# WanqingXia/UR-gym

Hardware: AMD Instinct MI355X
Metric: env-steps/sec (whole node) (higher is better)
Workload: dtype f64; 1 GPU; UR5DynReach-v1 N=65536 per GPU, random actions U(-1,1), auto-reset, seed 0; envs_total=65536, gather_obs=False, rollout_api=False, gjk_start=bullet

## Files before the change

ur_gym_amd/csrc/urgym_device.h:

```cpp
#pragma once
#include <stdint.h>
#if defined(URGYM_HOST_HARNESS)
#include <cmath>
#define __device__
#define __forceinline__ inline
#define URGYM_LDS
static inline uint32_t __umulhi(uint32_t a, uint32_t b) { return (uint32_t)(((uint64_t)a * b) >> 32); }
using std::fma; using std::sqrt; using std::fabs; using std::fmin; using std::fmax; using std::acos; using std::asin; using std::atan2;
#else
#include <hip/hip_runtime.h>
#define URGYM_LDS __attribute__((address_space(3)))
#endif
#include "urgym_philox.h"

namespace urgym {

struct D3 {
  double x, y, z;
};
__device__ __forceinline__ D3 d3(double x, double y, double z) { return D3{x, y, z}; }
__device__ __forceinline__ D3 operator+(D3 a, D3 b) { return d3(a.x + b.x, a.y + b.y, a.z + b.z); }
__device__ __forceinline__ D3 operator-(D3 a, D3 b) { return d3(a.x - b.x, a.y - b.y, a.z - b.z); }
__device__ __forceinline__ D3 operator-(D3 a) { return d3(-a.x, -a.y, -a.z); }
__device__ __forceinline__ D3 operator*(D3 a, double s) { return d3(a.x * s, a.y * s, a.z * s); }
__device__ __forceinline__ double dot(D3 a, D3 b) { return fma(a.x, b.x, fma(a.y, b.y, a.z * b.z)); }
__device__ __forceinline__ D3 cross(D3 a, D3 b) {
  return d3(a.y * b.z - a.z * b.y, a.z * b.x - a.x * b.z, a.x * b.y - a.y * b.x);
}
__device__ __forceinline__ double len2(D3 a) { return dot(a, a); }
__device__ __forceinline__ D3 sel(bool c, D3 a, D3 b) { return d3(c ? a.x : b.x, c ? a.y : b.y, c ? a.z : b.z); }

struct X3 {
  double r[9];
  D3 t;
};
__device__ __forceinline__ D3 rot(const X3& T, D3 v) {
  return d3(fma(T.r[0], v.x, fma(T.r[1], v.y, T.r[2] * v.z)), fma(T.r[3], v.x, fma(T.r[4], v.y, T.r[5] * v.z)),
            fma(T.r[6], v.x, fma(T.r[7], v.y, T.r[8] * v.z)));
}
__device__ __forceinline__ D3 rotT(const X3& T, D3 v) {
  return d3(fma(T.r[0], v.x, fma(T.r[3], v.y, T.r[6] * v.z)), fma(T.r[1], v.x, fma(T.r[4], v.y, T.r[7] * v.z)),
            fma(T.r[2], v.x, fma(T.r[5], v.y, T.r[8] * v.z)));
}
__device__ __forceinline__ D3 apply(const X3& T, D3 v) { return rot(T, v) + T.t; }
__device__ __forceinline__ X3 rel(const X3& A, const X3& B) {
  X3 C;
#pragma unroll
  for (int i = 0; i < 3; i++)
#pragma unroll
    for (int j = 0; j < 3; j++) C.r[i * 3 + j] = fma(A.r[i], B.r[j], fma(A.r[3 + i], B.r[3 + j], A.r[6 + i] * B.r[6 + j]));
  C.t = rotT(A, B.t - A.t);
  return C;
}

struct XRef {
  URGYM_LDS double* p;
  int stride;
  __device__ __forceinline__ double at(int k) const { return p[k * stride]; }
  __device__ __forceinline__ void set(int k, double v) const { p[k * stride] = v; }
};
__device__ __forceinline__ void store(XRef R, const X3& T) {
#pragma unroll
  for (int k = 0; k < 9; k++) R.set(k, T.r[k]);
  R.set(9, T.t.x); R.set(10, T.t.y); R.set(11, T.t.z);
}
__device__ __forceinline__ D3 rotT(XRef T, D3 v) {
  return d3(fma(T.at(0), v.x, fma(T.at(3), v.y, T.at(6) * v.z)), fma(T.at(1), v.x, fma(T.at(4), v.y, T.at(7) * v.z)),
            fma(T.at(2), v.x, fma(T.at(5), v.y, T.at(8) * v.z)));
}
__device__ __forceinline__ D3 apply(XRef T, D3 v) {
  return d3(fma(T.at(0), v.x, fma(T.at(1), v.y, T.at(2) * v.z)) + T.at(9), fma(T.at(3), v.x, fma(T.at(4), v.y, T.at(5) * v.z)) + T.at(10),
            fma(T.at(6), v.x, fma(T.at(7), v.y, T.at(8) * v.z)) + T.at(11));
}

struct Q4 {
  double x, y, z, w;
};
__device__ __forceinline__ Q4 qmul(Q4 a, Q4 b) {
  return Q4{a.w * b.x + a.x * b.w + a.y * b.z - a.z * b.y, a.w * b.y + a.y * b.w + a.z * b.x - a.x * b.z,
            a.w * b.z + a.z * b.w + a.x * b.y - a.y * b.x, a.w * b.w - a.x * b.x - a.y * b.y - a.z * b.z};
}
__device__ __forceinline__ void quat_to_rot(Q4 q, double r[9]) {
  double d = q.x * q.x + q.y * q.y + q.z * q.z + q.w * q.w;
  double s = 2.0 / d;
  double xs = q.x * s, ys = q.y * s, zs = q.z * s;
  double wx = q.w * xs, wy = q.w * ys, wz = q.w * zs, xx = q.x * xs, xy = q.x * ys, xz = q.x * zs;
  double yy = q.y * ys, yz = q.y * zs, zz = q.z * zs;
  r[0] = 1.0 - (yy + zz); r[1] = xy - wz; r[2] = xz + wy;
  r[3] = xy + wz; r[4] = 1.0 - (xx + zz); r[5] = yz - wx;
  r[6] = xz - wy; r[7] = yz + wx; r[8] = 1.0 - (xx + yy);
}
__device__ __forceinline__ Q4 rot_to_quat(const double r[9]) {
  double tr = r[0] + r[4] + r[8];
  Q4 q;
  if (tr > 0.0) {
    double s = sqrt(tr + 1.0);
    q.w = 0.5 * s;
    s = 0.5 / s;
    q.x = (r[7] - r[5]) * s; q.y = (r[2] - r[6]) * s; q.z = (r[3] - r[1]) * s;
  } else if (r[0] >= r[4] && r[0] >= r[8]) {
    double s = sqrt(r[0] - r[4] - r[8] + 1.0);
    q.x = 0.5 * s;
    s = 0.5 / s;
    q.w = (r[7] - r[5]) * s; q.y = (r[3] + r[1]) * s; q.z = (r[6] + r[2]) * s;
  } else if (r[4] >= r[8]) {
    double s = sqrt(r[4] - r[8] - r[0] + 1.0);
    q.y = 0.5 * s;
    s = 0.5 / s;
    q.w = (r[2] - r[6]) * s; q.z = (r[7] + r[5]) * s; q.x = (r[1] + r[3]) * s;
  } else {
    double s = sqrt(r[8] - r[0] - r[4] + 1.0);
    q.z = 0.5 * s;
    s = 0.5 / s;
    q.w = (r[3] - r[1]) * s; q.x = (r[2] + r[6]) * s; q.y = (r[5] + r[7]) * s;
  }
  return q;
}
__device__ __forceinline__ Q4 quat_from_rpy(double roll, double pitch, double yaw) {
  double sr, cr, sp, cp, sy, cy;
  sincos(0.5 * roll, &sr, &cr);
  sincos(0.5 * pitch, &sp, &cp);
  sincos(0.5 * yaw, &sy, &cy);
  return Q4{sr * cp * cy - cr * sp * sy, cr * sp * cy + sr * cp * sy, cr * cp * sy - sr * sp * cy, cr * cp * cy + sr * sp * sy};
}
__device__ __forceinline__ void rpy_from_quat(Q4 q, double& roll, double& pitch, double& yaw) {
  const double HALF_PI = 1.5707963267948966;
  double sarg = -2.0 * (q.x * q.z - q.w * q.y);
  if (sarg <= -0.99999) {
    roll = 0.0; pitch = -HALF_PI; yaw = 2.0 * atan2(q.x, -q.y);
  } else if (sarg >= 0.99999) {
    roll = 0.0; pitch = HALF_PI; yaw = 2.0 * atan2(-q.x, q.y);
  } else {
    double sqx = q.x * q.x, sqy = q.y * q.y, sqz = q.z * q.z, squ = q.w * q.w;
    roll = atan2(2.0 * (q.y * q.z + q.w * q.x), squ - sqx - sqy + sqz);
    pitch = asin(sarg);
    yaw = atan2(2.0 * (q.x * q.y + q.w * q.z), squ + sqx - sqy - sqz);
// ... 514 lines not shown
```

ur_gym_amd/csrc/urgym_hip.hip:

```cpp
#include <hip/hip_runtime.h>
#include <stdint.h>
#include <stdio.h>
#include <string.h>
#include <math.h>
#include <new>
#include <type_traits>
#include <vector>

#include "../../include/urgym.h"
#include "../../data/ur5e_model.h"
#include "urgym_device.h"
#include "urgym_handle.h"
#include "urgym_tables_host.h"

using namespace urgym;


namespace {

constexpr int WAVES = 4;
constexpr int THREADS = GROUP * WAVES;
constexpr uint32_t NO_ITEM = 0xFFFFFFFFu;
#ifndef URGYM_REFILL_MIN
#define URGYM_REFILL_MIN 16
#endif
constexpr int REFILL_MIN = URGYM_REFILL_MIN;
static_assert(REFILL_MIN >= 1 && REFILL_MIN <= 64, "a wave has 64 lanes");
constexpr int RESIDENT = 3;
constexpr int SC_ROWS = 19;
constexpr int LF_FIRST = 4, LF_LINKS = 3, LF_ROWS = 12 * LF_LINKS;
constexpr int PAIR_TABLE = 0, PAIR_TRACK = 5, PAIR_SELF = 10;
__host__ __device__ constexpr int self_pair_bit(int la, int lb) {
  return PAIR_SELF + (la == 1 ? 0 : (la == 2 ? 4 : 7)) + (lb - (la + 2));
}

enum { MODE_STEP = 0, MODE_RESET = 1, MODE_REFRESH = 2, MODE_PREFETCH = 3 };
enum { Q_TABLE = 0, Q_TRACK = 1, Q_SELF = 2 };

constexpr double M_HULL = 0.001, M_PRIM = 0.001;
constexpr double CYL_R = 0.05, CYL_H = 0.4, M_CYL = M_PRIM;
constexpr double TABLE_CX = 0.5, TABLE_CY = 0.0, TABLE_CZ = -0.58, TABLE_HX = 0.55, TABLE_HY = 0.9, TABLE_HZ = 0.46;
constexpr double M_TABLE = M_PRIM;
constexpr double TRACK_CX = 0.0, TRACK_CY = 0.0, TRACK_CZ = -0.06, TRACK_HX = 0.1, TRACK_HY = 0.55, TRACK_HZ = 0.06;
constexpr double M_TRACK = M_PRIM;
constexpr double TARGET_BOX_H = 0.025, M_TARGET_BOX = M_PRIM, TARGET_SPHERE_R = 0.02;

struct DevTables {
  double joint_rot[6][9];
  double joint_xyz[6][3];
  double capsule[6][7];
};
__constant__ DevTables c_tab;

constexpr int REC_FIELDS = 36;
enum { REC_GOAL = 0, REC_START = 6, REC_END = 12, REC_VEL = 18, REC_QUAT = 24, REC_LD = 28, REC_DP = 33 };

struct KParams {
  urgym_config cfg;
  urgym_buffers buf;
  HullMap graph;
  int obs_dim, goal_dim;
  uint32_t seed_lo, seed_hi;
  int pp;
  int copy_final;
  int envs;
  int big_blocks;
  int envs_tail;
  double* rec_d;
  int32_t* rec_i;
  int2* rlist;
  int* rcount;
  int rcap;
  double* ld_scratch;
  double* sc_scratch;
  double* lf_scratch;
  int* rzero;
  int* rzero2;
  int fallback_on;
  int prefetch;
  int inline_ori;
  float neutral_ach[6];
};
__device__ __forceinline__ double& REC(const KParams& P, int slot, int f, int n) {
  return P.rec_d[((size_t)slot * REC_FIELDS + f) * P.cfg.num_envs + n];
}
__device__ __forceinline__ int32_t& RECI(const KParams& P, int slot, int j, int n) {
  return P.rec_i[((size_t)slot * 2 + j) * P.cfg.num_envs + n];
}

__device__ __forceinline__ double& SOA(double* base, int f, int n, int N) { return base[(size_t)f * N + n]; }

__device__ __forceinline__ long long sortable(double x) {
  const long long k = __double_as_longlong(x);
  return k ^ ((k >> 63) & 0x7FFFFFFFFFFFFFFFLL);
}
__device__ __forceinline__ double unsortable(long long k) { return __longlong_as_double(k ^ ((k >> 63) & 0x7FFFFFFFFFFFFFFFLL)); }

__device__ __forceinline__ ShapeDesc hull_desc(int link ) {
  ShapeDesc s;
  s.type = SH_HULL; s.hull = link - 1; s.hx = s.hy = s.hz = 0.0;
  return s;
}
__device__ __forceinline__ ShapeDesc cyl_desc() {
  ShapeDesc s;
  s.type = SH_CYLZ; s.hull = 0;
  s.hx = s.hy = CYL_R - M_CYL; s.hz = 0.5 * CYL_H - M_CYL;
  return s;
}
__device__ __forceinline__ ShapeDesc box_desc(double hx, double hy, double hz, double margin) {
  ShapeDesc s;
  s.type = SH_BOX; s.hull = 0;
  s.hx = hx - margin; s.hy = hy - margin; s.hz = hz - margin;
  return s;
}
__device__ __forceinline__ ShapeDesc point_desc() {
  ShapeDesc s;
  s.type = SH_POINT; s.hull = 0; s.hx = s.hy = s.hz = 0.0;
  return s;
}

__device__ __forceinline__ void fk_joint(X3& T, int k, double s, double c) {
  const double* F = c_tab.joint_rot[k];
  const double* o = c_tab.joint_xyz[k];
  T.t = T.t + rot(T, d3(o[0], o[1], o[2]));
  double g[9];
#pragma unroll
  for (int i = 0; i < 3; i++) {
    g[i * 3 + 0] = F[i * 3 + 0] * c + F[i * 3 + 1] * s;
    g[i * 3 + 1] = F[i * 3 + 1] * c - F[i * 3 + 0] * s;
    g[i * 3 + 2] = F[i * 3 + 2];
  }
  double r[9];
#pragma unroll
  for (int i = 0; i < 3; i++)
#pragma unroll
    for (int j = 0; j < 3; j++) r[i * 3 + j] = fma(T.r[i * 3], g[j], fma(T.r[i * 3 + 1], g[3 + j], T.r[i * 3 + 2] * g[6 + j]));
#pragma unroll
  for (int i = 0; i < 9; i++) T.r[i] = r[i];
}
__device__ __forceinline__ X3 identity_x3() {
  X3 T;
  T.r[0] = 1; T.r[1] = 0; T.r[2] = 0; T.r[3] = 0; T.r[4] = 1; T.r[5] = 0; T.r[6] = 0; T.r[7] = 0; T.r[8] = 1;
  T.t = d3(0, 0, 0);
  return T;
}

__device__ __forceinline__ double segseg_dist(D3 p1, D3 q1, D3 p2, D3 q2) {
  D3 d1 = q1 - p1, d2 = q2 - p2, r = p1 - p2;
  double a = dot(d1, d1), e = dot(d2, d2), f = dot(d2, r);
  double s, t;
  const double EPS = 1e-18;
  if (a <= EPS && e <= EPS) return sqrt(len2(r));
  if (a <= EPS) {
    s = 0.0;
    t = fmin(1.0, fmax(0.0, f / e));
  } else {
    double c = dot(d1, r);
    if (e <= EPS) {
      t = 0.0;
      s = fmin(1.0, fmax(0.0, -c / a));
    } else {
      double b = dot(d1, d2), den = a * e - b * b;
      s = den > 1e-30 ? fmin(1.0, fmax(0.0, (b * f - c * e) / den)) : 0.0;
      t = (b * s + f) / e;
      if (t < 0.0) { t = 0.0; s = fmin(1.0, fmax(0.0, -c / a)); }
      else if (t > 1.0) { t = 1.0; s = fmin(1.0, fmax(0.0, (b - c) / a)); }
    }
  }
  D3 c1 = p1 + d1 * s, c2 = p2 + d2 * t;
  return sqrt(len2(c1 - c2));
}
__device__ __forceinline__ double seg_box_lower_bound(D3 p, D3 q, double cx, double cy, double cz, double hx, double hy, double hz) {
  double gx = fmax(fmax((cx - hx) - fmax(p.x, q.x), fmin(p.x, q.x) - (cx + hx)), 0.0);
  double gy = fmax(fmax((cy - hy) - fmax(p.y, q.y), fmin(p.y, q.y) - (cy + hy)), 0.0);
  double gz = fmax(fmax((cz - hz) - fmax(p.z, q.z), fmin(p.z, q.z) - (cz + hz)), 0.0);
  return sqrt(gx * gx + gy * gy + gz * gz);
}

__device__ void dyn_velocity(const double start[6], const double end[6], double T, double vel[6]) {
  for (int i = 0; i < 3; i++) vel[i] = (end[i] - start[i]) / T;
  Q4 q0 = quat_from_rpy(start[3], start[4], start[5]), q1 = quat_from_rpy(end[3], end[4], end[5]);
  double dm = (q0.x - q1.x) * (q0.x - q1.x) + (q0.y - q1.y) * (q0.y - q1.y) + (q0.z - q1.z) * (q0.z - q1.z) + (q0.w - q1.w) * (q0.w - q1.w);
  double dp = (q0.x + q1.x) * (q0.x + q1.x) + (q0.y + q1.y) * (q0.y + q1.y) + (q0.z + q1.z) * (q0.z + q1.z) + (q0.w + q1.w) * (q0.w + q1.w);
  if (!(dm < dp)) { q1.x = -q1.x; q1.y = -q1.y; q1.z = -q1.z; q1.w = -q1.w; }
  Q4 dq = qmul(q1, Q4{-q0.x, -q0.y, -q0.z, q0.w});
  double w = fmin(1.0, fmax(-1.0, dq.w));
  double angle = 2.0 * acos(w);
  double s2 = 1.0 - dq.w * dq.w;
  D3 axis = d3(1, 0, 0);
  if (!(s2 < 10.0 * 2.220446049250313e-16)) {
    double s = 1.0 / sqrt(s2);
    axis = d3(dq.x * s, dq.y * s, dq.z * s);
  }
  vel[3] = axis.x * angle / T; vel[4] = axis.y * angle / T; vel[5] = axis.z * angle / T;
}

__device__ __forceinline__ void step_displacement(const double vel[6], double dt, double dp[3]) {
  const double h = dt / 20.0;
  D3 v = d3(vel[0], vel[1], vel[2]);
  const D3 w = d3(vel[3], vel[4], vel[5]);
  double px = 0.0, py = 0.0, pz = 0.0;
#pragma unroll 1
  for (int k = 0; k < 20; k++) {
    v = v + cross(w, v) * h;
    px += h * v.x; py += h * v.y; pz += h * v.z;
  }
  dp[0] = px; dp[1] = py; dp[2] = pz;
}
__device__ __forceinline__ void integrate_obstacle(double pos[3], Q4& q, const double vel[6], const double dp[3], double dt) {
  pos[0] += dp[0]; pos[1] += dp[1]; pos[2] += dp[2];
  D3 w = d3(vel[3], vel[4], vel[5]);
  double ang = sqrt(len2(w));
  if (ang > 0.0) {
    double s, c;
    sincos(0.5 * ang * dt, &s, &c);
    double k = s / ang;
    Q4 dq{w.x * k, w.y * k, w.z * k, c};
    Q4 r = qmul(dq, q);
    double nrm = 1.0 / sqrt(r.x * r.x + r.y * r.y + r.z * r.z + r.w * r.w);
    q = Q4{r.x * nrm, r.y * nrm, r.z * nrm, r.w * nrm};
  }
}


__device__ __forceinline__ bool dyn_travel_ok(const KParams& P, int n, uint32_t episode, int attempt) {
  const urgym_config& cfg = P.cfg;
  uint32_t o1[4], o2[4], o3[4];
  philox4x32_10(P.seed_lo, P.seed_hi, (uint32_t)n, episode, (uint32_t)attempt, 1u, o1);
  philox4x32_10(P.seed_lo, P.seed_hi, (uint32_t)n, episode, (uint32_t)attempt, 2u, o2);
  philox4x32_10(P.seed_lo, P.seed_hi, (uint32_t)n, episode, (uint32_t)attempt, 3u, o3);
  const double us[3] = {u01(o1[1]), u01(o1[2]), u01(o1[3])};
  const double ue[3] = {u01(o2[3]), u01(o3[0]), u01(o3[1])};
  double dd[3];
#pragma unroll
  for (int i = 0; i < 3; i++) {
    const double a = cfg.obst_low[i] + (cfg.obst_high[i] - cfg.obst_low[i]) * us[i];
    const double b = cfg.obst_low[i] + (cfg.obst_high[i] - cfg.obst_low[i]) * ue[i];
    dd[i] = b - a;
  }
  const double d2 = dd[0] * dd[0] + dd[1] * dd[1] + dd[2] * dd[2];
  return !(sqrt(d2) < cfg.min_travel);
}

template <int KIND>
__device__ bool sample_attempt(const KParams& P, XRef slot, int n, uint32_t episode, int attempt, double goal[6], double st[6], double en[6]) {
  const urgym_config& cfg = P.cfg;
  const double DEG = 3.141592653589793 / 180.0;
    double u[20];
#pragma unroll
    for (int blk = 0; blk < 5; blk++) {
      uint32_t o[4];
      philox4x32_10(P.seed_lo, P.seed_hi, (uint32_t)n, episode, (uint32_t)attempt, (uint32_t)blk, o);
      u[blk * 4 + 0] = u01(o[0]); u[blk * 4 + 1] = u01(o[1]); u[blk * 4 + 2] = u01(o[2]); u[blk * 4 + 3] = u01(o[3]);
    }
#pragma unroll
    for (int i = 0; i < 3; i++) goal[i] = cfg.goal_low[i] + (cfg.goal_high[i] - cfg.goal_low[i]) * u[i];
    if (KIND != URGYM_ENV_OBS) {
      goal[3] = (-90.0 + (-180.0 - -90.0) * u[3]) * DEG;
      goal[4] = 0.0 * DEG;
      goal[5] = (0.0 + (-180.0 - 0.0) * u[4]) * DEG;
// ... 125 lines not shown
template <int KIND>
__device__ __forceinline__ void obstacle_of_step(const KParams& P, int n, double opos[3], Q4& oq) {
  const urgym_config& cfg = P.cfg;
  const urgym_buffers& B = P.buf;
  const int N = cfg.num_envs;
  for (int i = 0; i < 3; i++) opos[i] = SOA(B.obst_pos, i, n, N);
  oq = Q4{SOA(B.obst_quat, 0, n, N), SOA(B.obst_quat, 1, n, N), SOA(B.obst_quat, 2, n, N), SOA(B.obst_quat, 3, n, N)};
  if (KIND == URGYM_ENV_DYN && B.step_count[n] < cfg.dyn_motion_steps) {
    double ovel[6], dp[3];
    for (int i = 0; i < 6; i++) ovel[i] = SOA(B.obst_vel, i, n, N);
    for (int i = 0; i < 3; i++) dp[i] = SOA(B.obst_vel, 6 + i, n, N);
    integrate_obstacle(opos, oq, ovel, dp, cfg.dt);
  }
  if (KIND == URGYM_ENV_STA) {
    double st[6], en[6];
    bool moving = false;
    for (int i = 0; i < 6; i++) { st[i] = SOA(B.obst_start, i, n, N); en[i] = SOA(B.obst_end, i, n, N); moving = moving || en[i] != 0.0; }
    if (moving) {
      const double dx = en[0] - opos[0], dy = en[1] - opos[1], dz = en[2] - opos[2];
      double ovel[6] = {0, 0, 0, 0, 0, 0}, dp[3];
      if (sqrt(dx * dx + dy * dy + dz * dz) > 0.05) dyn_velocity(st, en, 1.0, ovel);
      step_displacement(ovel, cfg.dt, dp);
      integrate_obstacle(opos, oq, ovel, dp, cfg.dt);
    }
  }
}

template <int MODE>
struct EnvLds {
  static constexpr int ME = (MODE == MODE_PREFETCH) ? PREFETCH_MAX_ENVS : ((MODE == MODE_STEP) ? STEP_MAX_ENVS : MAX_ENVS);
  static constexpr bool LDS_Q = (MODE == MODE_REFRESH);
  static constexpr bool DIST_LDS = (MODE != MODE_STEP);
  static constexpr bool LDS_STATE = (MODE != MODE_STEP);
  double s_dist[5][DIST_LDS ? ME : 1];
  double s_q[LDS_Q ? 6 : 1][LDS_Q ? ME : 1];
  double s_obst[LDS_STATE ? 7 : 1][LDS_STATE ? ME : 1];
  uint32_t s_pairs[ME];
  int s_flags[ME];
  int s_env[ME];
  alignas(16) int s_ticket;
  int s_pending;
  int s_p1done;
  int s_left;
  int s_key[(MODE != MODE_STEP) ? ME : 1];
  double s_kind[(MODE == MODE_STEP) ? 8 : 1][5];
  double s_pose[GJK_SLOT_DOUBLES][THREADS];
};

template <int KIND, int MODE, bool WITH_EPA>
__device__ __forceinline__ void env_body(const KParams& P, const float* __restrict__ actions, EnvLds<MODE>& L, const int bidx, const int nblk) {
  constexpr int ME = EnvLds<MODE>::ME;
  constexpr bool LDS_Q = EnvLds<MODE>::LDS_Q, DIST_LDS = EnvLds<MODE>::DIST_LDS, LDS_STATE = EnvLds<MODE>::LDS_STATE;
  auto& s_dist = L.s_dist;
  auto& s_q = L.s_q;
  auto& s_obst = L.s_obst;
  auto& s_pairs = L.s_pairs;
  auto& s_flags = L.s_flags;
  auto& s_env = L.s_env;
  int& s_ticket = L.s_ticket;
  int& s_pending = L.s_pending;
  int& s_p1done = L.s_p1done;
  int& s_left = L.s_left;
  auto& s_key = L.s_key;
  auto& s_pose = L.s_pose;

  const urgym_config& cfg = P.cfg;
  const urgym_buffers& B = P.buf;
  const int N = cfg.num_envs;
  const int tid = threadIdx.x;
  const int lane = tid & 63;
  const int wv = __builtin_amdgcn_readfirstlane(tid >> 6);
  constexpr int OD = (KIND == URGYM_ENV_ORI) ? 18 : ((KIND == URGYM_ENV_OBS) ? 26 : ((KIND == URGYM_ENV_STA) ? 29 : 35));
  constexpr int GD = (KIND == URGYM_ENV_OBS) ? 3 : 6;
  int vb = bidx;
  if (MODE == MODE_STEP && P.envs_tail == 0) {
    const int nb = nblk, x = vb & 7, per = nb >> 3, rem = nb & 7;
    vb = x * per + (x < rem ? x : rem) + (vb >> 3);
  }
  const bool tail_block = (MODE == MODE_STEP) && P.envs_tail > 0 && vb >= P.big_blocks;
  const int E = tail_block ? P.envs_tail : P.envs;
  const int first = tail_block ? P.big_blocks * P.envs + (vb - P.big_blocks) * P.envs_tail : vb * P.envs;
  const int G = (E + GROUP - 1) / GROUP;
  constexpr bool HAS_OBST = (KIND != URGYM_ENV_ORI);
  constexpr int COLL_BIT = 1 << 30;
  constexpr int EE_BIT = 1 << 29;
  constexpr int EPA_SHIFT = 8, EPA_MASK = 0x7FFF << EPA_SHIFT;
  const bool need_epa = WITH_EPA && ((KIND == URGYM_ENV_OBS) || !cfg.check_collision || (MODE != MODE_STEP));
  XRef pose_slot{(URGYM_LDS double*)&s_pose[0][0] + tid, THREADS};
  float* const s_out = reinterpret_cast<float*>(&s_pose[0][0]);
  static_assert(sizeof(float) * STEP_MAX_ENVS * 47 <= sizeof(double) * GJK_SLOT_DOUBLES * THREADS, "staging must fit");
  auto dist_cell = [&](int i, int e) -> double* {
    return DIST_LDS ? (double*)&s_dist[i][DIST_LDS ? e : 0] : &P.ld_scratch[(size_t)i * N + first + e];
  };

  if (bidx == 0 && tid == 0) {
    if (P.rzero) *P.rzero = 0;
    if (P.rzero2) *P.rzero2 = 0;
  }
  int list_count = 0;
  if (MODE != MODE_STEP) {
    list_count = (MODE == MODE_PREFETCH) ? min(*P.rcount, P.rcap) : B.done_count[P.pp];
    if (first >= list_count) return;
  }
  if (tid == 0) { s_ticket = THREADS; s_pending = 0; s_p1done = 0; s_left = 0; }
  if (MODE == MODE_STEP && tid < 8) {
    const int k = tid & 3, ex = tid >> 2;
    const bool tbl = (k == Q_TABLE);
    const double msum = M_HULL + ((k == 3) ? M_CYL : ((k == Q_SELF) ? M_HULL : (tbl ? M_TABLE : M_TRACK)));
    const bool wants = (k == 3) || ex;
    const double verdict = wants ? 0.0 : msum + cfg.collision_margin;
    L.s_kind[tid][0] = (k == 3) ? (CYL_R - M_CYL) : (tbl ? (TABLE_HX - M_TABLE) : (TRACK_HX - M_TRACK));
    L.s_kind[tid][1] = (k == 3) ? (CYL_R - M_CYL) : (tbl ? (TABLE_HY - M_TABLE) : (TRACK_HY - M_TRACK));
    L.s_kind[tid][2] = (k == 3) ? (0.5 * CYL_H - M_CYL) : (tbl ? (TABLE_HZ - M_TABLE) : (TRACK_HZ - M_TRACK));
    L.s_kind[tid][3] = wants ? msum + 0.02 + 5.0 : verdict;
    L.s_kind[tid][4] = verdict;
  }
  const bool workbench = (KIND != URGYM_ENV_ORI) && cfg.link_dist_scope == URGYM_LINK_DIST_WORKBENCH;
  if (workbench && tid < E && (DIST_LDS || first + tid < N))
    for (int i = 0; i < 5; i++) *dist_cell(i, tid) = __longlong_as_double(0x7FF0000000000000LL);
  if (MODE == MODE_STEP && tid < E) {
    s_env[tid] = (first + tid < N) ? first + tid : -1;
    s_flags[tid] = 0;
    s_pairs[tid] = 0;
  }
  const bool frames_on = (MODE == MODE_STEP) && HAS_OBST && !WITH_EPA && cfg.check_collision && (workbench ? 15 : 5) * E > THREADS;
  __syncthreads();
  const int p1_slot = (MODE == MODE_STEP) ? (wv - (WAVES - G)) * GROUP + lane : lane;
  const bool p1_lane = ((MODE == MODE_STEP) ? (wv >= WAVES - G) : (wv == 0)) && (p1_slot < E);
  int n_slot = -1, flags_slot = 0;
  int key_slot = 0;
  if (p1_lane) {
    const int idx = first + p1_slot;
    if (MODE == MODE_STEP) n_slot = idx < N ? idx : -1;
    else if (MODE == MODE_PREFETCH) {
      if (idx < list_count) { const int2 ent = P.rlist[idx]; n_slot = ent.x; key_slot = ent.y; }
    } else n_slot = idx < list_count ? B.done_list[idx] : -1;
  }
  if ((MODE == MODE_RESET || MODE == MODE_PREFETCH) && wv == 0) {
    int episode_used = 0;
    sample_episode_wave<KIND>(P, pose_slot, E, lane, n_slot, key_slot, MODE == MODE_PREFETCH, flags_slot, episode_used);
    if (p1_lane) s_key[p1_slot] = (MODE == MODE_PREFETCH) ? key_slot : episode_used + 1;
  }
  if (p1_lane) {
    const int e = p1_slot;
    const int n = n_slot;
    int flags = flags_slot;
    double q[6] = {0, 0, 0, 0, 0, 0};
    double opos[3] = {0, 0, 0};
    Q4 oq{0, 0, 0, 1};
    bool finite = true;
    if (n >= 0) {
      for (int i = 0; i < 6; i++) q[i] = joint_of_step<MODE>(P, actions, n, i);
      for (int i = 0; i < 6; i++) finite = finite && (fabs(q[i]) < 1.0e6);
      if (MODE == MODE_STEP) {
        bool over = false;
        for (int i = 0; i < 6; i++) over = over || (fabs(q[i]) > (i == 2 ? 3.141592653589793 : 6.283185307179586));
        if (over) atomicOr(&s_flags[p1_slot], URGYM_STATUS_JOINT_LIMIT);
      }
      if (HAS_OBST && LDS_STATE) {
        double sp[6];
        for (int i = 0; i < 6; i++) sp[i] = (MODE == MODE_PREFETCH) ? REC(P, key_slot & 1, REC_START + i, n) : SOA(B.obst_start, i, n, N);
        for (int i = 0; i < 3; i++) opos[i] = sp[i];
        oq = quat_from_rpy(sp[3], sp[4], sp[5]);
      }
    }
    const bool live = (n >= 0 && finite);
    const bool use_cache = (MODE == MODE_STEP) && (HAS_OBST || cfg.check_collision);
    if (use_cache && live) {
#pragma unroll 1
      for (int k = 0; k < 6; k++) {
        double sn, cs;
        sincos(joint_of_step<MODE>(P, actions, n, k), &sn, &cs);
        SOA(P.sc_scratch, 2 * k, n, N) = sn;
        SOA(P.sc_scratch, 2 * k + 1, n, N) = cs;
      }
      if (HAS_OBST) {
        obstacle_of_step<KIND>(P, n, opos, oq);
        for (int i = 0; i < 3; i++) SOA(P.sc_scratch, 12 + i, n, N) = opos[i];
        SOA(P.sc_scratch, 15, n, N) = oq.x; SOA(P.sc_scratch, 16, n, N) = oq.y; SOA(P.sc_scratch, 17, n, N) = oq.z; SOA(P.sc_scratch, 18, n, N) = oq.w;
      }
    }
    s_env[e] = live ? n : (n >= 0 ? -2 - n : -1);
    if (MODE != MODE_STEP) s_flags[e] = flags;
    if (LDS_STATE) {
      if (LDS_Q) for (int i = 0; i < 6; i++) s_q[i][e] = q[i];
      s_obst[0][e] = opos[0]; s_obst[1][e] = opos[1]; s_obst[2][e] = opos[2];
      s_obst[3][e] = oq.x; s_obst[4][e] = oq.y; s_obst[5][e] = oq.z; s_obst[6][e] = oq.w;
    }
    if (HAS_OBST && !live && (DIST_LDS || n >= 0))
      for (int i = 0; i < 5; i++) *dist_cell(i, e) = (n >= 0) ? __builtin_nan("") : 1e30;
    uint32_t pairs = 0;
    if (live && cfg.check_collision && MODE != MODE_RESET && MODE != MODE_PREFETCH) {
      const double lim = cfg.collision_margin + M_HULL + 1e-6;
      X3 T = identity_x3();
      D3 a0[3], a1[3];
      double sn45[2] = {0, 0}, cs45[2] = {0, 0};
#pragma unroll
      for (int k = 0; k < 6; k++) {
        double sn, cs;
        if (frames_on && k >= LF_FIRST) { sn = sn45[k - LF_FIRST]; cs = cs45[k - LF_FIRST]; }
        else if (use_cache) { sn = SOA(P.sc_scratch, 2 * k, n, N); cs = SOA(P.sc_scratch, 2 * k + 1, n, N); }
        else sincos(q[k], &sn, &cs);
        fk_joint(T, k, sn, cs);
        const int link = k + 1;
        if (frames_on && link == LF_FIRST)
          for (int j = 0; j < 2; j++) { sn45[j] = SOA(P.sc_scratch, 2 * (LF_FIRST + j), n, N); cs45[j] = SOA(P.sc_scratch, 2 * (LF_FIRST + j) + 1, n, N); }
        if (frames_on && link >= LF_FIRST) {
          const int row = 12 * (link - LF_FIRST);
          for (int i = 0; i < 9; i++) SOA(P.lf_scratch, row + i, n, N) = T.r[i];
          SOA(P.lf_scratch, row + 9, n, N) = T.t.x; SOA(P.lf_scratch, row + 10, n, N) = T.t.y; SOA(P.lf_scratch, row + 11, n, N) = T.t.z;
        }
        const double* c = c_tab.capsule[k];
        const D3 b0 = apply(T, d3(c[0], c[1], c[2])), b1 = apply(T, d3(c[3], c[4], c[5]));
        const double rb = c[6];
        if (k < 3) { a0[k] = b0; a1[k] = b1; }
        if (link >= 2) {
          if (seg_box_lower_bound(b0, b1, TABLE_CX, TABLE_CY, TABLE_CZ, TABLE_HX, TABLE_HY, TABLE_HZ) - rb <= lim) pairs |= 1u << (PAIR_TABLE + link - 2);
          if (seg_box_lower_bound(b0, b1, TRACK_CX, TRACK_CY, TRACK_CZ, TRACK_HX, TRACK_HY, TRACK_HZ) - rb <= lim) pairs |= 1u << (PAIR_TRACK + link - 2);
        }
#pragma unroll
        for (int A = 1; A <= 3; A++) {
          if (A <= link - 2) {
            if (segseg_dist(a0[A - 1], a1[A - 1], b0, b1) - c_tab.capsule[A - 1][6] - rb <= lim + M_HULL) pairs |= 1u << self_pair_bit(A, link);
          }
        }
      }
      if (MODE == MODE_STEP) {
        double er, ep, ey;
        rpy_from_quat(rot_to_quat(T.r), er, ep, ey);
        float* orow = B.observation + (size_t)n * OD;
        orow[0] = (float)T.t.x; orow[1] = (float)T.t.y; orow[2] = (float)T.t.z;
        orow[3] = (float)er; orow[4] = (float)ep; orow[5] = (float)ey;
        atomicOr(&s_flags[e], EE_BIT);
      }
    }
    s_pairs[e] = pairs;
    if (pairs) atomicAdd(&s_pending, __popc(pairs));
  }
  if (MODE == MODE_STEP) {
    if (wv >= WAVES - G && lane == 0) __hip_atomic_fetch_add(&s_p1done, 1, __ATOMIC_RELEASE, __HIP_MEMORY_SCOPE_WORKGROUP);
  } else {
    __syncthreads();
  }

  if (!(MODE == MODE_STEP && !HAS_OBST && !cfg.check_collision)) {
    D3 v0 = d3(0, 1, 0);
    int kind = 3, e = 0, lb = 2, la = 1;
    auto shape_a = [&]() -> ShapeDesc { return hull_desc(kind == Q_SELF ? la : lb); };
    auto shape_b = [&]() -> ShapeDesc {
      ShapeDesc s;
      s.type = (kind == 3) ? SH_CYLZ : ((kind == Q_SELF) ? SH_HULL : SH_BOX);
      s.hull = lb - 1;
      const bool tbl = (kind == Q_TABLE);
      s.hx = (kind == 3) ? (CYL_R - M_CYL) : (tbl ? (TABLE_HX - M_TABLE) : (TRACK_HX - M_TRACK));
      s.hy = (kind == 3) ? (CYL_R - M_CYL) : (tbl ? (TABLE_HY - M_TABLE) : (TRACK_HY - M_TRACK));
      s.hz = (kind == 3) ? (0.5 * CYL_H - M_CYL) : (tbl ? (TABLE_HZ - M_TABLE) : (TRACK_HZ - M_TRACK));
      return s;
    };
    bool exact = false;
    const bool guided = cfg.gjk_start == URGYM_GJK_START_GUIDED;
    auto capsule_mid = [&](int link, const X3& TX) -> D3 {
      const double* c = c_tab.capsule[link - 1];
      return apply(TX, d3(0.5 * (c[0] + c[3]), 0.5 * (c[1] + c[4]), 0.5 * (c[2] + c[5])));
    };
    auto guided_axis = [&](D3 mid, D3 centre) -> D3 {
      const D3 d = mid - centre;
      const double n2 = dot(d, d);
      return n2 > 1e-12 ? d * (1.0 / sqrt(n2)) : d3(0, 1, 0);
    };
    bool p1_ok = (MODE != MODE_STEP);
    auto setup = [&](uint32_t item, auto after_p1) -> bool {
      e = item & 255;
      kind = (item >> 8) & 3;
      exact = ((item >> 16) & 1) != 0;
      lb = (item >> 10) & 7;
      la = (item >> 13) & 7;
      if (e >= E || lb < 1 || lb > 6 || (kind == Q_SELF && (la < 1 || la > 6))) return false;
      const int n = s_env[e];
      if (n < 0) return false;
      const bool cached = (MODE == MODE_STEP) && (decltype(after_p1)::value || p1_ok);
      if (MODE == MODE_STEP && !cached) {
        bool finite = true;
        for (int k = 0; k < 6; k++) finite = finite && (fabs(joint_of_step<MODE>(P, actions, n, k)) < 1.0e6);
        if (!finite) return false;
      }
      X3 T = identity_x3(), TA = identity_x3();
      const bool framed = decltype(after_p1)::value && frames_on && lb >= LF_FIRST && kind != Q_SELF;
      auto load_frame = [&]() {
        const int row = 12 * (lb - LF_FIRST);
        for (int i = 0; i < 9; i++) T.r[i] = SOA(P.lf_scratch, row + i, n, N);
        T.t = d3(SOA(P.lf_scratch, row + 9, n, N), SOA(P.lf_scratch, row + 10, n, N), SOA(P.lf_scratch, row + 11, n, N));
      };
#pragma unroll 1
      for (int k = 0; k < (framed ? 0 : lb); k++) {
        double sn, cs;
        if (cached) { sn = SOA(P.sc_scratch, 2 * k, n, N); cs = SOA(P.sc_scratch, 2 * k + 1, n, N); }
        else sincos(LDS_Q ? s_q[k][e] : joint_of_step<MODE>(P, actions, n, k), &sn, &cs);
        fk_joint(T, k, sn, cs);
        if (k + 1 == la) TA = T;
      }
      if (kind == 3) {
        X3 To;
        if (LDS_STATE) {
          quat_to_rot(Q4{s_obst[3][e], s_obst[4][e], s_obst[5][e], s_obst[6][e]}, To.r);
          To.t = d3(s_obst[0][e], s_obst[1][e], s_obst[2][e]);
        } else if (cached) {
          quat_to_rot(Q4{SOA(P.sc_scratch, 15, n, N), SOA(P.sc_scratch, 16, n, N), SOA(P.sc_scratch, 17, n, N), SOA(P.sc_scratch, 18, n, N)}, To.r);
          To.t = d3(SOA(P.sc_scratch, 12, n, N), SOA(P.sc_scratch, 13, n, N), SOA(P.sc_scratch, 14, n, N));
        } else {
          double op[3];
          Q4 oqs;
          obstacle_of_step<KIND>(P, n, op, oqs);
          quat_to_rot(oqs, To.r);
          To.t = d3(op[0], op[1], op[2]);
        }
        if (framed) load_frame();
        store(pose_slot, rel(To, T));
        v0 = rotT(To, guided ? guided_axis(capsule_mid(lb, T), To.t) : d3(0, 1, 0));
      } else if (kind == Q_SELF) {
        store(pose_slot, rel(T, TA));
        v0 = rotT(T, guided ? guided_axis(capsule_mid(la, TA), capsule_mid(lb, T)) : d3(0, 1, 0));
      } else {
        if (framed) load_frame();
        const bool tbl = (kind == Q_TABLE);
        const D3 centre = d3(tbl ? TABLE_CX : TRACK_CX, tbl ? TABLE_CY : TRACK_CY, tbl ? TABLE_CZ : TRACK_CZ);
        v0 = guided ? guided_axis(capsule_mid(lb, T), centre) : d3(0, 1, 0);
        T.t = T.t - centre;
        store(pose_slot, T);
      }
      return true;
    };
    auto claim_pair = [&]() -> uint32_t {
      int pe = tid % E;
#pragma unroll 1
      for (int trip = 0; trip < 2 * ME; trip++, pe = (pe + 1 == E ? 0 : pe + 1)) {
        uint32_t m = s_pairs[pe];
        while (m) {
          const int b = __ffs((int)m) - 1;
          const uint32_t old = atomicAnd(&s_pairs[pe], ~(1u << b));
          if (old & (1u << b)) {
            if (b < PAIR_TRACK) return (uint32_t)pe | (Q_TABLE << 8) | ((uint32_t)(b - PAIR_TABLE + 2) << 10);
            if (b < PAIR_SELF) return (uint32_t)pe | (Q_TRACK << 8) | ((uint32_t)(b - PAIR_TRACK + 2) << 10);
            const int i = b - PAIR_SELF;
            const int la = i < 4 ? 1 : (i < 7 ? 2 : 3);
            const int l2 = i < 4 ? 3 + i : (i < 7 ? i : i - 2);
            return (uint32_t)pe | (Q_SELF << 8) | ((uint32_t)l2 << 10) | ((uint32_t)la << 13);
          }
          m = old & ~(1u << b);
        }
      }
      return NO_ITEM;
    };
    auto margin_sum = [&]() -> double {
      return M_HULL + ((kind == 3) ? M_CYL : ((kind == Q_SELF) ? M_HULL : ((kind == Q_TABLE) ? M_TABLE : M_TRACK)));
    };
    const int n_tickets = HAS_OBST ? (workbench ? 15 : 5) * E : 0;
    auto ticket_item = [&](int t) -> uint32_t {
      const int body = t / (5 * E), r = t - body * 5 * E;
      const int tl = r / E, te = r - tl * E, link = 2 + tl;
      if (body == 0) return (uint32_t)te | (3u << 8) | ((uint32_t)link << 10);
      return (uint32_t)te | ((uint32_t)(body == 1 ? Q_TABLE : Q_TRACK) << 8) | ((uint32_t)link << 10) | (1u << 16);
    };

    GjkRun run;
    run.info = 0;
    bool busy = false;
    if (MODE == MODE_STEP) p1_ok = __hip_atomic_load(&s_p1done, __ATOMIC_ACQUIRE, __HIP_MEMORY_SCOPE_WORKGROUP) >= G;
    if (tid < n_tickets) {
      busy = setup(ticket_item(tid), std::false_type{});
      if (busy) gjk_begin(run, v0);
    }
    auto file_distance = [&](double dist) {
      if (workbench) atomicMin(reinterpret_cast<long long*>(dist_cell(lb - 2, e)), sortable(dist));
      else *dist_cell(lb - 2, e) = dist;
    };
    auto file_overlap = [&]() {
      const double msum = margin_sum();
      const int body = (kind == 3) ? 0 : (kind == Q_TABLE ? 1 : 2);
      atomicOr(&s_flags[e], URGYM_STATUS_PENETRATION | (need_epa ? (1 << (EPA_SHIFT + 5 * body + (lb - 2))) : 0));
      file_distance(-msum);
    };
    auto file = [&]() {
      if (!busy && (run.info & GJK_FIN_MASK)) {
        const int fin = run.info >> GJK_FIN_SHIFT;
        run.info &= ~GJK_FIN_MASK;
        gjk_finish(run, !(fin & 2), (fin & 4) != 0);
        const double msum = margin_sum();
        if (kind == 3 || exact) {
          if (run.info & GJK_ITERCAP) atomicOr(&s_flags[e], URGYM_STATUS_GJK_ITER);
          if (run.info & GJK_PENETRATING) file_overlap();
          else file_distance(run.core - msum);
        } else {
          const bool hit = (run.info & (GJK_PENETRATING | GJK_CLOSE)) || (!(run.info & GJK_SEPARATED) && (run.core - msum) <= cfg.collision_margin);
          if (hit) atomicOr(&s_flags[e], COLL_BIT);
        }
        run.info = 0;
      }
    };
    auto trip = [&]() __attribute__((always_inline)) {
      if (busy) {
        int fin;
        if (MODE == MODE_STEP) {
          const URGYM_LDS double* row = (const URGYM_LDS double*)(URGYM_LDS void*)&L.s_kind[kind | ((int)exact << 2)][0];
          ShapeDesc sb;
          sb.type = (kind == 3) ? SH_CYLZ : ((kind == Q_SELF) ? SH_HULL : SH_BOX);
          sb.hull = lb - 1;
          sb.hx = row[0]; sb.hy = row[1]; sb.hz = row[2];
          fin = gjk_advance(run, P.graph, shape_a(), pose_slot, sb, row[3], row[4]);
        } else {
          const bool wants_distance = (kind == 3 || exact);
          const double verdict_d = wants_distance ? 0.0 : margin_sum() + cfg.collision_margin;
          fin = gjk_advance(run, P.graph, shape_a(), pose_slot, shape_b(), wants_distance ? margin_sum() + 0.02 + 5.0 : verdict_d, verdict_d);
        }
        if (fin) {
          run.info |= fin << GJK_FIN_SHIFT;
          busy = false;
          if (HAS_OBST && WITH_EPA) {
            if (need_epa && (kind == 3 || exact) && gjk_ends_penetrating(run, fin)) {
              file_overlap();
              run.info = 0;
            }
          }
        }
      }
    };
    for (;;) {
      do trip(); while (__popcll(__ballot(!busy)) < REFILL_MIN);
      typedef int pool_words __attribute__((ext_vector_type(4)));
      const pool_words pool = *(volatile URGYM_LDS pool_words*)(URGYM_LDS void*)&s_ticket;
      __builtin_amdgcn_fence(__ATOMIC_ACQUIRE, "workgroup");
      const bool more_tickets = pool.x < n_tickets;
      const bool p1_published = (MODE != MODE_STEP) || pool.z >= G;
      const bool more_pairs = pool.y > 0;
      if (MODE == MODE_STEP) p1_ok = p1_published;
      if (!busy && p1_ok) {
        file();
        uint32_t item = NO_ITEM;
        if (more_tickets) {
          const int t = atomicAdd(&s_ticket, 1);
          if (t < n_tickets) item = ticket_item(t);
        } else if (more_pairs) {
          if (atomicSub(&s_pending, 1) > 0) item = claim_pair();
        }
        if (item != NO_ITEM) {
          busy = setup(item, std::true_type{});
          if (busy) gjk_begin(run, v0);
        }
      }
      if (!more_tickets && !more_pairs && p1_published) {
        bool dry = true;
// ... 1018 lines not shown
```

Baseline: 350.4 million env-steps/s.

## Add phase-1 head tweaks: squared-distance culls, in-pass sincos, bounded publish wait

Three step-mode changes, each behind a compile-time bit flag and all on by default. The culling tests compare squared distances against a squared bound with a small slack instead of taking sqrt. When collision checking is on, sincos is computed inside the FK pass instead of in a separate pre-pass over global scratch, and the later reload of the joint 4 and 5 values is dropped. Waves that process tickets may now poll briefly with s_sleep until phase 1 has published its frames, so ticket setup can load cached link frames instead of recomputing FK. The wait can stall waves, and the squared cull slack can change borderline culling decisions.

```diff
diff --git a/ur_gym_amd/csrc/urgym_device.h b/ur_gym_amd/csrc/urgym_device.h
--- a/ur_gym_amd/csrc/urgym_device.h
+++ b/ur_gym_amd/csrc/urgym_device.h
@@ -52,6 +52,44 @@
   C.t = rotT(A, B.t - A.t);
   return C;
 }
+
+__device__ __forceinline__ double segseg_dist2(D3 p1, D3 q1, D3 p2, D3 q2) {
+  D3 d1 = q1 - p1, d2 = q2 - p2, r = p1 - p2;
+  double a = dot(d1, d1), e = dot(d2, d2), f = dot(d2, r);
+  double s, t;
+  const double EPS = 1e-18;
+  if (a <= EPS && e <= EPS) return len2(r);
+  if (a <= EPS) {
+    s = 0.0;
+    t = fmin(1.0, fmax(0.0, f / e));
+  } else {
+    double c = dot(d1, r);
+    if (e <= EPS) {
+      t = 0.0;
+      s = fmin(1.0, fmax(0.0, -c / a));
+    } else {
+      double b = dot(d1, d2), den = a * e - b * b;
+      s = den > 1e-30 ? fmin(1.0, fmax(0.0, (b * f - c * e) / den)) : 0.0;
+      t = (b * s + f) / e;
+      if (t < 0.0) { t = 0.0; s = fmin(1.0, fmax(0.0, -c / a)); }
+      else if (t > 1.0) { t = 1.0; s = fmin(1.0, fmax(0.0, (b - c) / a)); }
+    }
+  }
+  D3 c1 = p1 + d1 * s, c2 = p2 + d2 * t;
+  return len2(c1 - c2);
+}
+__device__ __forceinline__ double segseg_dist(D3 p1, D3 q1, D3 p2, D3 q2) { return sqrt(segseg_dist2(p1, q1, p2, q2)); }
+__device__ __forceinline__ double seg_box_lower_bound2(D3 p, D3 q, double cx, double cy, double cz, double hx, double hy, double hz) {
+  double gx = fmax(fmax((cx - hx) - fmax(p.x, q.x), fmin(p.x, q.x) - (cx + hx)), 0.0);
+  double gy = fmax(fmax((cy - hy) - fmax(p.y, q.y), fmin(p.y, q.y) - (cy + hy)), 0.0);
+  double gz = fmax(fmax((cz - hz) - fmax(p.z, q.z), fmin(p.z, q.z) - (cz + hz)), 0.0);
+  return gx * gx + gy * gy + gz * gz;
+}
+__device__ __forceinline__ double seg_box_lower_bound(D3 p, D3 q, double cx, double cy, double cz, double hx, double hy, double hz) {
+  return sqrt(seg_box_lower_bound2(p, q, cx, cy, cz, hx, hy, hz));
+}
+constexpr double CULL_SLACK = 1e-12;
+__device__ __forceinline__ double cull_bound2(double reach) { return (reach * reach) * (1.0 + CULL_SLACK); }
 
 struct XRef {
   URGYM_LDS double* p;
diff --git a/ur_gym_amd/csrc/urgym_hip.hip b/ur_gym_amd/csrc/urgym_hip.hip
--- a/ur_gym_amd/csrc/urgym_hip.hip
+++ b/ur_gym_amd/csrc/urgym_hip.hip
@@ -25,6 +25,9 @@
 #define URGYM_REFILL_MIN 16
 #endif
 constexpr int REFILL_MIN = URGYM_REFILL_MIN;
+#ifndef URGYM_HEAD_ITEMS
+#define URGYM_HEAD_ITEMS 7
+#endif
 static_assert(REFILL_MIN >= 1 && REFILL_MIN <= 64, "a wave has 64 lanes");
 constexpr int RESIDENT = 3;
 constexpr int SC_ROWS = 19;
@@ -145,37 +148,6 @@
   return T;
 }
 
-__device__ __forceinline__ double segseg_dist(D3 p1, D3 q1, D3 p2, D3 q2) {
-  D3 d1 = q1 - p1, d2 = q2 - p2, r = p1 - p2;
-  double a = dot(d1, d1), e = dot(d2, d2), f = dot(d2, r);
-  double s, t;
-  const double EPS = 1e-18;
-  if (a <= EPS && e <= EPS) return sqrt(len2(r));
-  if (a <= EPS) {
-    s = 0.0;
-    t = fmin(1.0, fmax(0.0, f / e));
-  } else {
-    double c = dot(d1, r);
-    if (e <= EPS) {
-      t = 0.0;
-      s = fmin(1.0, fmax(0.0, -c / a));
-    } else {
-      double b = dot(d1, d2), den = a * e - b * b;
-      s = den > 1e-30 ? fmin(1.0, fmax(0.0, (b * f - c * e) / den)) : 0.0;
-      t = (b * s + f) / e;
-      if (t < 0.0) { t = 0.0; s = fmin(1.0, fmax(0.0, -c / a)); }
-      else if (t > 1.0) { t = 1.0; s = fmin(1.0, fmax(0.0, (b - c) / a)); }
-    }
-  }
-  D3 c1 = p1 + d1 * s, c2 = p2 + d2 * t;
-  return sqrt(len2(c1 - c2));
-}
-__device__ __forceinline__ double seg_box_lower_bound(D3 p, D3 q, double cx, double cy, double cz, double hx, double hy, double hz) {
-  double gx = fmax(fmax((cx - hx) - fmax(p.x, q.x), fmin(p.x, q.x) - (cx + hx)), 0.0);
-  double gy = fmax(fmax((cy - hy) - fmax(p.y, q.y), fmin(p.y, q.y) - (cy + hy)), 0.0);
-  double gz = fmax(fmax((cz - hz) - fmax(p.z, q.z), fmin(p.z, q.z) - (cz + hz)), 0.0);
-  return sqrt(gx * gx + gy * gy + gz * gz);
-}
 
 __device__ void dyn_velocity(const double start[6], const double end[6], double T, double vel[6]) {
   for (int i = 0; i < 3; i++) vel[i] = (end[i] - start[i]) / T;
@@ -467,6 +439,8 @@
   const int first = tail_block ? P.big_blocks * P.envs + (vb - P.big_blocks) * P.envs_tail : vb * P.envs;
   const int G = (E + GROUP - 1) / GROUP;
   constexpr bool HAS_OBST = (KIND != URGYM_ENV_ORI);
+  constexpr bool HEAD = (MODE == MODE_STEP) && !WITH_EPA;
+  constexpr bool HEAD_WAIT = HEAD && (URGYM_HEAD_ITEMS & 1), HEAD_SQ = HEAD && (URGYM_HEAD_ITEMS & 2), HEAD_REG = HEAD && (URGYM_HEAD_ITEMS & 4);
   constexpr int COLL_BIT = 1 << 30;
   constexpr int EE_BIT = 1 << 29;
   constexpr int EPA_SHIFT = 8, EPA_MASK = 0x7FFF << EPA_SHIFT;
@@ -551,13 +525,17 @@
     }
     const bool live = (n >= 0 && finite);
     const bool use_cache = (MODE == MODE_STEP) && (HAS_OBST || cfg.check_collision);
+    bool sincos_in_pass = false;
+    if constexpr (HEAD_REG) sincos_in_pass = live && cfg.check_collision;
     if (use_cache && live) {
+      if (!sincos_in_pass) {
 #pragma unroll 1
-      for (int k = 0; k < 6; k++) {
-        double sn, cs;
-        sincos(joint_of_step<MODE>(P, actions, n, k), &sn, &cs);
-        SOA(P.sc_scratch, 2 * k, n, N) = sn;
-        SOA(P.sc_scratch, 2 * k + 1, n, N) = cs;
+        for (int k = 0; k < 6; k++) {
+          double sn, cs;
+          sincos(joint_of_step<MODE>(P, actions, n, k), &sn, &cs);
+          SOA(P.sc_scratch, 2 * k, n, N) = sn;
+          SOA(P.sc_scratch, 2 * k + 1, n, N) = cs;
+        }
       }
       if (HAS_OBST) {
         obstacle_of_step<KIND>(P, n, opos, oq);
@@ -583,12 +561,16 @@
 #pragma unroll
       for (int k = 0; k < 6; k++) {
         double sn, cs;
-        if (frames_on && k >= LF_FIRST) { sn = sn45[k - LF_FIRST]; cs = cs45[k - LF_FIRST]; }
+        if constexpr (HEAD_REG) {
+          sincos(q[k], &sn, &cs);
+          SOA(P.sc_scratch, 2 * k, n, N) = sn;
+          SOA(P.sc_scratch, 2 * k + 1, n, N) = cs;
+        } else if (frames_on && k >= LF_FIRST) { sn = sn45[k - LF_FIRST]; cs = cs45[k - LF_FIRST]; }
         else if (use_cache) { sn = SOA(P.sc_scratch, 2 * k, n, N); cs = SOA(P.sc_scratch, 2 * k + 1, n, N); }
         else sincos(q[k], &sn, &cs);
         fk_joint(T, k, sn, cs);
         const int link = k + 1;
-        if (frames_on && link == LF_FIRST)
+        if (!HEAD_REG && frames_on && link == LF_FIRST)
           for (int j = 0; j < 2; j++) { sn45[j] = SOA(P.sc_scratch, 2 * (LF_FIRST + j), n, N); cs45[j] = SOA(P.sc_scratch, 2 * (LF_FIRST + j) + 1, n, N); }
         if (frames_on && link >= LF_FIRST) {
           const int row = 12 * (link - LF_FIRST);
@@ -600,13 +582,23 @@
         const double rb = c[6];
         if (k < 3) { a0[k] = b0; a1[k] = b1; }
         if (link >= 2) {
-          if (seg_box_lower_bound(b0, b1, TABLE_CX, TABLE_CY, TABLE_CZ, TABLE_HX, TABLE_HY, TABLE_HZ) - rb <= lim) pairs |= 1u << (PAIR_TABLE + link - 2);
-          if (seg_box_lower_bound(b0, b1, TRACK_CX, TRACK_CY, TRACK_CZ, TRACK_HX, TRACK_HY, TRACK_HZ) - rb <= lim) pairs |= 1u << (PAIR_TRACK + link - 2);
+          if constexpr (HEAD_SQ) {
+            const double box2 = cull_bound2(lim + rb);
+            if (seg_box_lower_bound2(b0, b1, TABLE_CX, TABLE_CY, TABLE_CZ, TABLE_HX, TABLE_HY, TABLE_HZ) <= box2) pairs |= 1u << (PAIR_TABLE + link - 2);
+            if (seg_box_lower_bound2(b0, b1, TRACK_CX, TRACK_CY, TRACK_CZ, TRACK_HX, TRACK_HY, TRACK_HZ) <= box2) pairs |= 1u << (PAIR_TRACK + link - 2);
+          } else {
+            if (seg_box_lower_bound(b0, b1, TABLE_CX, TABLE_CY, TABLE_CZ, TABLE_HX, TABLE_HY, TABLE_HZ) - rb <= lim) pairs |= 1u << (PAIR_TABLE + link - 2);
+            if (seg_box_lower_bound(b0, b1, TRACK_CX, TRACK_CY, TRACK_CZ, TRACK_HX, TRACK_HY, TRACK_HZ) - rb <= lim) pairs |= 1u << (PAIR_TRACK + link - 2);
+          }
         }
 #pragma unroll
         for (int A = 1; A <= 3; A++) {
           if (A <= link - 2) {
-            if (segseg_dist(a0[A - 1], a1[A - 1], b0, b1) - c_tab.capsule[A - 1][6] - rb <= lim + M_HULL) pairs |= 1u << self_pair_bit(A, link);
+            if constexpr (HEAD_SQ) {
+              if (segseg_dist2(a0[A - 1], a1[A - 1], b0, b1) <= cull_bound2(lim + M_HULL + c_tab.capsule[A - 1][6] + rb)) pairs |= 1u << self_pair_bit(A, link);
+            } else {
+              if (segseg_dist(a0[A - 1], a1[A - 1], b0, b1) - c_tab.capsule[A - 1][6] - rb <= lim + M_HULL) pairs |= 1u << self_pair_bit(A, link);
+            }
           }
         }
       }
@@ -670,7 +662,9 @@
         if (!finite) return false;
       }
       X3 T = identity_x3(), TA = identity_x3();
-      const bool framed = decltype(after_p1)::value && frames_on && lb >= LF_FIRST && kind != Q_SELF;
+      bool published = decltype(after_p1)::value;
+      if constexpr (HEAD_WAIT) published = published || p1_ok;
+      const bool framed = published && frames_on && lb >= LF_FIRST && kind != Q_SELF;
       auto load_frame = [&]() {
         const int row = 12 * (lb - LF_FIRST);
         for (int i = 0; i < 9; i++) T.r[i] = SOA(P.lf_scratch, row + i, n, N);
@@ -751,6 +745,16 @@
     run.info = 0;
     bool busy = false;
     if (MODE == MODE_STEP) p1_ok = __hip_atomic_load(&s_p1done, __ATOMIC_ACQUIRE, __HIP_MEMORY_SCOPE_WORKGROUP) >= G;
+    if constexpr (HEAD_WAIT) {
+      constexpr int P1_WAIT_POLLS = 32;
+      if (G > 1 && wv >= WAVES - G) {
+#pragma unroll 1
+        for (int poll = 0; poll < P1_WAIT_POLLS && !p1_ok; poll++) {
+          __builtin_amdgcn_s_sleep(2);
+          p1_ok = __builtin_amdgcn_readfirstlane(__hip_atomic_load(&s_p1done, __ATOMIC_ACQUIRE, __HIP_MEMORY_SCOPE_WORKGROUP)) >= G;
+        }
+      }
+    }
     if (tid < n_tickets) {
       busy = setup(ticket_item(tid), std::false_type{});
       if (busy) gjk_begin(run, v0);
```

Measured after the change: 354.3 million env-steps/s (median of 6 runs). +1.1%, better.
